# bharatlytics/faceRecognition_InfrenceEngine

Measured on AMD Instinct MI355X. Metric: faces/sec end-to-end @1080p, higher is better.
Workload: dtype f16

## Files before the change

### facerecognition_infrenceengine_amd/csrc/conv_walk64.hip

```cpp
#include "common.h"
#include <type_traits>

namespace {

constexpr int K64_RW = 28, K64_RH = 14, K64_C = 64;
constexpr int K64_PX = K64_RW * K64_RH;
constexpr int K64_HALO = 512 * 128;
constexpr int K64_SLOT = 64 * 128;
constexpr int K64_RING = 2 * K64_HALO, K64_PRMO = K64_RING + 3 * K64_SLOT;
constexpr int K64_PRM = 10 * 64 * 4;
constexpr int K64_LDS = K64_PRMO + K64_PRM;

struct Walk64P {
    const half_t* x; const half_t* w; half_t* y;
    const float* bias; const float* slope; const half_t* res;
    int B, HW, Cout, bias_mode;
    int nsplit;
    unsigned xbytes, ybytes, wbytes;
};

}

__global__ __launch_bounds__(512, 2) void conv_walk64_kernel(Walk64P p) {
#if defined(__HIP_DEVICE_COMPILE__)
    extern __shared__ __attribute__((aligned(16))) char lds[];
    char* ring = lds + K64_RING;
    float* lprm = reinterpret_cast<float*>(lds + K64_PRMO);
    const int tid = threadIdx.x;
    const int wave = __builtin_amdgcn_readfirstlane(tid >> 6);
    const int ncg = p.Cout >> 6;
    const int cg = blockIdx.x % ncg, part = (blockIdx.x / ncg) % p.nsplit, n = blockIdx.x / (ncg * p.nsplit);
    const int HW = p.HW, nbx = HW / K64_RW;
    const int reg0 = part * (nbx * (HW / K64_RH) / p.nsplit), nreg = reg0 + nbx * (HW / K64_RH) / p.nsplit;

    __amdgpu_buffer_rsrc_t wrs = buffer_rsrc(p.w, p.wbytes);
    __amdgpu_buffer_rsrc_t xrs = buffer_rsrc(p.x, p.xbytes);

    const unsigned wbase = (unsigned)cg * (9 * K64_SLOT);
    unsigned wq = 0;
    auto issue_w = [&](int slot, int ln) {
        __builtin_amdgcn_raw_ptr_buffer_load_lds(wrs, (lds_ptr_t)(ring + slot * K64_SLOT + wave * 1024), 16,
                                                 (unsigned)(wave * 1024 + ln * 16), wbase + wq * K64_SLOT, 0, 0);
        wq = wq == 8 ? 0 : wq + 1;
    };
    auto halo_lane = [&](int ln, bool left_edge, bool right_edge) -> unsigned {
        const int lrow = ln >> 3, ch = ln & 7, q = wave & 3;
        const unsigned out = (unsigned)((q == 0) & (lrow == 0) & left_edge) | (unsigned)((q == 3) & (lrow == 5) & right_edge) |
                             (unsigned)((q == 3) & (lrow >= 6));
        return ((unsigned)((lrow - 1) * 128 + ((ch ^ ((lrow + 4 * ((wave >> 2) & 1)) & 7)) << 4)) & (out - 1u)) | (out << 31);
    };
    auto issue_halo = [&](int buf, int i, int reg, int ln) {
        int n_ = n;
        asm volatile("" : "+s"(n_));
        const int by = reg / nbx, bx_ = reg - by * nbx;
        const int y0 = by * K64_RH, x0 = bx_ * K64_RW;
        const unsigned lt = halo_lane(ln, x0 == 0, x0 + K64_RW == HW);
        const int hy = 2 * i + (wave >> 2), iy = y0 - 1 + hy;
        const bool ok = reg < nreg && (unsigned)iy < (unsigned)HW;
        const unsigned so = (unsigned)(((n_ * HW + iy) * HW + x0 + (wave & 3) * 8) * 128);
        __builtin_amdgcn_raw_ptr_buffer_load_lds(xrs, (lds_ptr_t)(lds + buf * K64_HALO + (hy * 4 + (wave & 3)) * 1024), 16,
                                                 ok ? lt + so : 0x80000000u, 0, 0, 0);
    };

    {
        const int ln = tid & 63;
        issue_w(0, ln);
        issue_w(1, ln);
        issue_w(2, ln);
        for (int i = 0; i < 8; ++i) issue_halo(reg0 & 1, i, reg0, ln);
        for (int e = tid; e < 640; e += 512) {
            const int r = e >> 6, c = e & 63;
            float v;
            if (r < 9) v = p.bias ? p.bias[(p.bias_mode == 1 ? r * p.Cout : 0) + cg * 64 + c] : 0.f;
            else v = p.slope ? p.slope[cg * 64 + c] : 1.f;
            lprm[e] = v;
        }
    }

    float4v acc[3][4], accx;
    int4v a0[2][4], a1[2][4], b[3][2], bx[2];
    int boff[4];

    auto run = [&](auto role_tag) {
    constexpr int ROLE = decltype(role_tag)::value;
#pragma unroll 1
    for (int reg = reg0; reg < nreg; ++reg) {
        const int cur = reg & 1;
        int lane = tid & 63;
        asm volatile("" : "+v"(lane));
        const int fr = lane & 15, fq = lane >> 4;
        const int by = reg / nbx, bx_ = reg - by * nbx;
        const int y0 = by * K64_RH, x0 = bx_ * K64_RW;
        auto gpix = [&](int px) {
            const int oy = px / K64_RW, ox = px - oy * K64_RW;
            return (unsigned)((n * HW + y0 + oy) * HW + x0 + ox);
        };
        auto cls_off = [&](int px) {
            const int oy = px / K64_RW, ox = px - oy * K64_RW, ho = y0 + oy, wo = x0 + ox;
            return ((ho == 0 ? 0 : (ho == HW - 1 ? 2 : 1)) * 3 + (wo == 0 ? 0 : (wo == HW - 1 ? 2 : 1))) * 64;
        };
        auto ct = [&](int f) { return (f + wave) & 3; };
        auto co8 = [&](int ip) { return ct(2 * ip + (fq & 1)) * 16 + (fq >> 1) * 8; };
        int a_own = fr * 128 + ((fq ^ (fr & 7)) << 4);
        asm volatile("" : "+v"(a_own));
        int hb[3];
#pragma unroll
        for (int t = 0; t < 3; ++t) {
            const int px = (wave * 3 + t) * 16 + fr;
            const int oy = px / K64_RW, ox = px - oy * K64_RW;
            hb[t] = (oy + 1) * 32 + ox + 1;
            asm volatile("" : "+v"(hb[t]));
        }
        auto set_tap_one = [&](int t, int dy, int dx) {
            int l_ = lane;
            asm volatile("" : "+v"(l_));
            const int h = (t < 3 ? hb[t < 3 ? t : 0] : ((l_ & 15) < 8 ? 14 * 32 + 21 + (l_ & 15) : 33)) + dy * 32 + dx;
            boff[t] = cur * K64_HALO + h * 128 + (((l_ >> 4) ^ ((((h >> 3) & 4) + h) & 7)) << 4);
        };
        auto rd_a = [&](int slot, int kh, int i) { return *reinterpret_cast<const int4v*>(ring + slot * K64_SLOT + ct(i) * 2048 + (kh ? (a_own ^ 64) : a_own)); };
        auto rd_b = [&](int kh, int t) { return *reinterpret_cast<const int4v*>(lds + (kh ? (boff[t] ^ 64) : boff[t])); };

        asm volatile("s_waitcnt lgkmcnt(0)" ::: "memory");
        if (reg == reg0) __builtin_amdgcn_s_barrier();
#pragma unroll
        for (int t = 0; t < 3; ++t) {
            const int cj = cls_off((wave * 3 + t) * 16 + fr);
#pragma unroll
            for (int i = 0; i < 4; ++i) acc[t][i] = *reinterpret_cast<const float4v*>(lprm + cj + ct(i) * 16 + fq * 4);
        }
        accx = *reinterpret_cast<const float4v*>(lprm + cls_off(fr < 8 ? 384 + fr : 0) + (wave & 3) * 16 + fq * 4);
        if (p.res) {
            __amdgpu_buffer_rsrc_t rrs = buffer_rsrc(p.res, p.ybytes);
            int4v r[3][2];
#pragma unroll
            for (int t = 0; t < 3; ++t)
#pragma unroll
                for (int ip = 0; ip < 2; ++ip)
                    r[t][ip] = __builtin_bit_cast(int4v, __builtin_amdgcn_raw_buffer_load_b128(
                        rrs, (gpix((wave * 3 + t) * 16 + fr) * (unsigned)p.Cout + (unsigned)(cg * 64 + co8(ip))) * 2u, 0, 16));
            const int2v rx = __builtin_bit_cast(int2v, __builtin_amdgcn_raw_buffer_load_b64(
                rrs, fr < 8 ? (gpix(384 + fr) * (unsigned)p.Cout + (unsigned)(cg * 64 + (wave & 3) * 16 + fq * 4)) * 2u : 0x80000000u, 0, 16));
#pragma unroll
            for (int t = 0; t < 3; ++t)
#pragma unroll
                for (int ip = 0; ip < 2; ++ip) {
                    const auto s0 = __builtin_amdgcn_permlane16_swap((unsigned)r[t][ip][0], (unsigned)r[t][ip][2], false, false);
                    const auto s1 = __builtin_amdgcn_permlane16_swap((unsigned)r[t][ip][1], (unsigned)r[t][ip][3], false, false);
                    const half4 ha = __builtin_bit_cast(half4, int2v{(int)s0[0], (int)s1[0]});
                    const half4 hb_ = __builtin_bit_cast(half4, int2v{(int)s0[1], (int)s1[1]});
#pragma unroll
                    for (int e = 0; e < 4; ++e) { acc[t][2 * ip][e] += (float)ha[e]; acc[t][2 * ip + 1][e] += (float)hb_[e]; }
                }
            const half4 hx = __builtin_bit_cast(half4, rx);
#pragma unroll
            for (int e = 0; e < 4; ++e) accx[e] += (float)hx[e];
        }
        asm volatile("s_waitcnt vmcnt(0)" ::: "memory");
        __builtin_amdgcn_s_barrier();

#pragma unroll
        for (int t = 0; t < 4; ++t) set_tap_one(t, -1, -1);
#pragma unroll
        for (int kh = 0; kh < 2; ++kh) {
#pragma unroll
            for (int i = 0; i < 4; ++i) a0[kh][i] = rd_a(0, kh, i);
#pragma unroll
            for (int t = 0; t < 3; ++t) b[t][kh] = rd_b(kh, t);
            bx[kh] = rd_b(kh, 3);
        }

        auto step = [&](int4v (&ac)[2][4], int4v (&an)[2][4], int s) {
            const int nslot = (s + 1) % 3;
            const int tn = s + 1 < 9 ? s + 1 : 0;
            const int dyn = tn / 3 - 1, dxn = tn % 3 - 1;
            auto dma = [&]() {
                if (s < 8) issue_halo(cur ^ 1, s, reg + 1, lane);
                issue_w(s % 3, lane);
            };
            if constexpr (ROLE == 0) { dma(); FR_PIN(); }
#pragma unroll
            for (int kh = 0; kh < 2; ++kh) {
                accx = mfma16(ac[kh][0], bx[kh], accx);
                FR_PIN();
#pragma unroll
                for (int t = 0; t < 3; ++t) {
#pragma unroll
                    for (int i = 0; i < 4; ++i) acc[t][i] = mfma16(ac[kh][i], b[t][kh], acc[t][i]);
                    if (kh == 0) { an[0][t] = rd_a(nslot, 0, t); if (t == 2) an[0][3] = rd_a(nslot, 0, 3); }
                    else { an[1][t] = rd_a(nslot, 1, t); if (t == 2) an[1][3] = rd_a(nslot, 1, 3); }
                    if (kh == 0) set_tap_one(t, dyn, dxn);
                    b[t][kh] = rd_b(kh, t);
                    if (t == 2) {
                        if (kh == 0) set_tap_one(3, dyn, dxn);
                        bx[kh] = rd_b(kh, 3);
                    }
                    FR_PIN();
                }
                if constexpr (ROLE == 1) { if (kh == 0) { dma(); FR_PIN(); } }
            }
        };
#pragma unroll
        for (int s = 0; s < 9; ++s) {
            asm volatile("s_waitcnt vmcnt(2) lgkmcnt(1)" ::: "memory");
            __builtin_amdgcn_s_barrier();
            FR_PIN();
            if ((s & 1) == 0) step(a0, a1, s); else step(a1, a0, s);
        }

        asm volatile("s_waitcnt lgkmcnt(0)" ::: "memory");
        int le = lane;
        asm volatile("" : "+v"(le));
        const int fre = le & 15, fqe = le >> 4;
        float4v sv[4];
#pragma unroll
        for (int i = 0; i < 4; ++i) sv[i] = *reinterpret_cast<const float4v*>(lprm + 9 * 64 + ct(i) * 16 + fqe * 4);
        auto act = [&](float4v v, const float4v& s_) {
#pragma unroll
            for (int e = 0; e < 4; ++e) v[e] = v[e] > 0.f ? v[e] : v[e] * s_[e];
            return __builtin_bit_cast(int2v, half4{(half_t)v[0], (half_t)v[1], (half_t)v[2], (half_t)v[3]});
        };
        half_t* yo = p.y + cg * 64;
#pragma unroll
        for (int t = 0; t < 3; ++t) {
            const size_t gp = (size_t)gpix((wave * 3 + t) * 16 + fre) * p.Cout;
#pragma unroll
            for (int ip = 0; ip < 2; ++ip) {
                const int2v pa = act(acc[t][2 * ip], sv[2 * ip]), pb = act(acc[t][2 * ip + 1], sv[2 * ip + 1]);
                const auto s0 = __builtin_amdgcn_permlane16_swap((unsigned)pa[0], (unsigned)pb[0], false, false);
                const auto s1 = __builtin_amdgcn_permlane16_swap((unsigned)pa[1], (unsigned)pb[1], false, false);
                *reinterpret_cast<int4v*>(yo + gp + ct(2 * ip + (fqe & 1)) * 16 + (fqe >> 1) * 8) = int4v{(int)s0[0], (int)s1[0], (int)s0[1], (int)s1[1]};
            }
        }
        if (wave < 4 && fre < 8)
            *reinterpret_cast<int2v*>(yo + (size_t)gpix(384 + fre) * p.Cout + wave * 16 + fqe * 4) = act(accx, sv[0]);
    }
    };
    if ((wave >> 2) == 0) run(std::integral_constant<int, 0>{}); else run(std::integral_constant<int, 1>{});
    asm volatile("s_waitcnt vmcnt(0) lgkmcnt(0)" ::: "memory");
#endif
}

extern "C" size_t fr_conv_walk64_weight_bytes(int Cout) { return Cout > 0 ? (size_t)(Cout / 64) * 9 * K64_SLOT : 0; }

__global__ void walk64_pack_weights(const half_t* __restrict__ w, half_t* __restrict__ out, int ncg) {
    const int e = blockIdx.x * blockDim.x + threadIdx.x;
    if (e >= ncg * 9 * 512) return;
    const int q_ = e / 512, r = e - q_ * 512, row = r >> 3, cp = r & 7;
    const int cgi = q_ / 9, tap = q_ - cgi * 9;
    const int chunk = cp ^ (row & 7);
    const int4v v = *reinterpret_cast<const int4v*>(w + (size_t)(cgi * 64 + row) * 576 + tap * 64 + chunk * 8);
    *reinterpret_cast<int4v*>(out + (size_t)q_ * 4096 + row * 64 + cp * 8) = v;
}

extern "C" int fr_conv_walk64_pack(const void* w, void* out, int Cout, fr_stream_t stream) {
    FR_REQUIRE(w && out && Cout > 0 && Cout % 64 == 0, "fr_conv_walk64_pack: bad argument (Cout %d)", Cout);
    const int ncg = Cout / 64;
    walk64_pack_weights<<<fr_cdiv((int64_t)ncg * 9 * 512, 256), 256, 0, fr_stream(stream)>>>((const half_t*)w, (half_t*)out, ncg);
    FR_CHECK_LAUNCH("walk64_pack_weights");
    return FR_OK;
}

extern "C" int fr_conv_walk64_f16(const void* x, const void* wstream, void* y, const float* bias, int bias_mode, const float* slope,
                                  const void* residual, int B, int HW, int Cout, fr_stream_t stream) {
    FR_REQUIRE(x && wstream && y && B > 0, "fr_conv_walk64_f16: bad argument");
    FR_REQUIRE(x != y, "fr_conv_walk64_f16: y must not alias x");
    FR_REQUIRE(HW > 0 && HW % 28 == 0 && Cout > 0 && Cout % 64 == 0, "fr_conv_walk64_f16: image side %d must be a multiple of 28, Cout %d of 64", HW, Cout);
    FR_REQUIRE(bias_mode == 0 || bias_mode == 1, "fr_conv_walk64_f16: bad bias_mode");
    FR_REQUIRE((int64_t)B * HW * HW * 64 * 2 < (1ll << 31) && (int64_t)B * HW * HW * Cout * 2 < (1ll << 32),
               "fr_conv_walk64_f16: tensor too large for 32-bit buffer offsets (split the batch)");
    Walk64P p;
    p.x = (const half_t*)x; p.w = (const half_t*)wstream; p.y = (half_t*)y;
    p.bias = bias; p.slope = slope; p.res = (const half_t*)residual;
    p.B = B; p.HW = HW; p.Cout = Cout; p.bias_mode = bias_mode;
    const int nregs = (HW / 28) * (HW / 14);
    p.nsplit = 1;
    while (p.nsplit < 8 && (int64_t)B * (Cout / 64) * p.nsplit * 2 <= 256 && nregs % (p.nsplit * 2) == 0 && nregs / (p.nsplit * 2) >= 2) p.nsplit *= 2;
    p.xbytes = (unsigned)((int64_t)B * HW * HW * 64 * 2);
    p.ybytes = (unsigned)((int64_t)B * HW * HW * Cout * 2);
    p.wbytes = (unsigned)((int64_t)(Cout / 64) * 9 * K64_SLOT);
    static FrDevLatch latch;
    if (!fr_raise_lds(reinterpret_cast<const void*>(conv_walk64_kernel), K64_LDS, latch)) {
        fr_set_error("fr_conv_walk64_f16: cannot raise dynamic LDS to %d bytes", K64_LDS);
        return FR_E_LAUNCH;
    }
    conv_walk64_kernel<<<B * (Cout / 64) * p.nsplit, 512, K64_LDS, fr_stream(stream)>>>(p);
    FR_CHECK_LAUNCH("conv_walk64_kernel");
    return FR_OK;
}
```

Measured before the change: 26950.

## Keep conv weights resident in registers instead of streaming through LDS ring

Each wave now loads its half of the output-channel weight fragments for all 9 taps into VGPRs once at kernel start, removing the per-tap LDS weight ring, its DMA issues and the per-step barriers. Work is re-split so waves partition pixels by group (6 tiles each) and channels by half, with the extra 8 pixels handled by two pixel groups, and the weight pack layout changes to per-lane MFMA fragments. This trades a large register footprint (36 int4 per lane) for fewer LDS reads and synchronisation, which may hurt occupancy at two blocks per CU.

Result: no change. 26870 (-0.3%).

```diff
diff --git a/facerecognition_infrenceengine_amd/csrc/conv_walk64.hip b/facerecognition_infrenceengine_amd/csrc/conv_walk64.hip
--- a/facerecognition_infrenceengine_amd/csrc/conv_walk64.hip
+++ b/facerecognition_infrenceengine_amd/csrc/conv_walk64.hip
@@ -6,10 +6,11 @@
 constexpr int K64_RW = 28, K64_RH = 14, K64_C = 64;
 constexpr int K64_PX = K64_RW * K64_RH;
 constexpr int K64_HALO = 512 * 128;
-constexpr int K64_SLOT = 64 * 128;
-constexpr int K64_RING = 2 * K64_HALO, K64_PRMO = K64_RING + 3 * K64_SLOT;
+constexpr int K64_PRMO = 2 * K64_HALO;
 constexpr int K64_PRM = 10 * 64 * 4;
 constexpr int K64_LDS = K64_PRMO + K64_PRM;
+constexpr int K64_FRAG = 64 * 16;
+constexpr int K64_WCG = 4 * 9 * 2 * K64_FRAG;
 
 struct Walk64P {
     const half_t* x; const half_t* w; half_t* y;
@@ -24,25 +25,17 @@
 __global__ __launch_bounds__(512, 2) void conv_walk64_kernel(Walk64P p) {
 #if defined(__HIP_DEVICE_COMPILE__)
     extern __shared__ __attribute__((aligned(16))) char lds[];
-    char* ring = lds + K64_RING;
     float* lprm = reinterpret_cast<float*>(lds + K64_PRMO);
     const int tid = threadIdx.x;
     const int wave = __builtin_amdgcn_readfirstlane(tid >> 6);
+    const int pg = wave & 3, hf = wave >> 2;
     const int ncg = p.Cout >> 6;
     const int cg = blockIdx.x % ncg, part = (blockIdx.x / ncg) % p.nsplit, n = blockIdx.x / (ncg * p.nsplit);
     const int HW = p.HW, nbx = HW / K64_RW;
     const int reg0 = part * (nbx * (HW / K64_RH) / p.nsplit), nreg = reg0 + nbx * (HW / K64_RH) / p.nsplit;
 
-    __amdgpu_buffer_rsrc_t wrs = buffer_rsrc(p.w, p.wbytes);
     __amdgpu_buffer_rsrc_t xrs = buffer_rsrc(p.x, p.xbytes);
 
-    const unsigned wbase = (unsigned)cg * (9 * K64_SLOT);
-    unsigned wq = 0;
-    auto issue_w = [&](int slot, int ln) {
-        __builtin_amdgcn_raw_ptr_buffer_load_lds(wrs, (lds_ptr_t)(ring + slot * K64_SLOT + wave * 1024), 16,
-                                                 (unsigned)(wave * 1024 + ln * 16), wbase + wq * K64_SLOT, 0, 0);
-        wq = wq == 8 ? 0 : wq + 1;
-    };
     auto halo_lane = [&](int ln, bool left_edge, bool right_edge) -> unsigned {
         const int lrow = ln >> 3, ch = ln & 7, q = wave & 3;
         const unsigned out = (unsigned)((q == 0) & (lrow == 0) & left_edge) | (unsigned)((q == 3) & (lrow == 5) & right_edge) |
@@ -62,12 +55,20 @@
                                                  ok ? lt + so : 0x80000000u, 0, 0, 0);
     };
 
+    int4v wf[2][9][2];
     {
         const int ln = tid & 63;
-        issue_w(0, ln);
-        issue_w(1, ln);
-        issue_w(2, ln);
         for (int i = 0; i < 8; ++i) issue_halo(reg0 & 1, i, reg0, ln);
+        __amdgpu_buffer_rsrc_t wrs = buffer_rsrc(p.w, p.wbytes);
+        const unsigned wbase = (unsigned)cg * K64_WCG + (unsigned)hf * (K64_WCG / 2);
+#pragma unroll
+        for (int c = 0; c < 2; ++c)
+#pragma unroll
+            for (int tap = 0; tap < 9; ++tap)
+#pragma unroll
+                for (int kh = 0; kh < 2; ++kh)
+                    wf[c][tap][kh] = __builtin_bit_cast(int4v, __builtin_amdgcn_raw_buffer_load_b128(
+                        wrs, (unsigned)(ln * 16), wbase + (unsigned)(((c * 9 + tap) * 2 + kh) * K64_FRAG), 0));
         for (int e = tid; e < 640; e += 512) {
             const int r = e >> 6, c = e & 63;
             float v;
@@ -77,16 +78,17 @@
         }
     }
 
-    float4v acc[3][4], accx;
-    int4v a0[2][4], a1[2][4], b[3][2], bx[2];
-    int boff[4];
+    float4v acc[6][2], accx;
+    int4v b[7];
+    int boff[7];
 
     auto run = [&](auto role_tag) {
-    constexpr int ROLE = decltype(role_tag)::value;
+    constexpr int XF = decltype(role_tag)::value;
+    constexpr int NT = XF < 2 ? 7 : 6;
 #pragma unroll 1
     for (int reg = reg0; reg < nreg; ++reg) {
         const int cur = reg & 1;
-        int lane = tid & 63;
+        int lane = (int)__builtin_amdgcn_mbcnt_hi(~0u, __builtin_amdgcn_mbcnt_lo(~0u, 0u));
         asm volatile("" : "+v"(lane));
         const int fr = lane & 15, fq = lane >> 4;
         const int by = reg / nbx, bx_ = reg - by * nbx;
@@ -99,121 +101,102 @@
             const int oy = px / K64_RW, ox = px - oy * K64_RW, ho = y0 + oy, wo = x0 + ox;
             return ((ho == 0 ? 0 : (ho == HW - 1 ? 2 : 1)) * 3 + (wo == 0 ? 0 : (wo == HW - 1 ? 2 : 1))) * 64;
         };
-        auto ct = [&](int f) { return (f + wave) & 3; };
-        auto co8 = [&](int ip) { return ct(2 * ip + (fq & 1)) * 16 + (fq >> 1) * 8; };
-        int a_own = fr * 128 + ((fq ^ (fr & 7)) << 4);
-        asm volatile("" : "+v"(a_own));
-        int hb[3];
-#pragma unroll
-        for (int t = 0; t < 3; ++t) {
-            const int px = (wave * 3 + t) * 16 + fr;
+        auto co8 = [&]() { return (2 * hf + (fq & 1)) * 16 + (fq >> 1) * 8; };
+        auto tile_px = [&](int t) { return (pg * 6 + t) * 16 + fr; };
+        auto haddr = [&](int h) { return cur * K64_HALO + h * 128 + ((((h >> 3) & 4) + h) & 7) * 16; };
+        auto rd_b = [&](int t, int fx) { return *reinterpret_cast<const int4v*>(lds + (boff[t] ^ fx)); };
+
+        auto init_acc = [&](auto res_tag) {
+            constexpr bool RES = decltype(res_tag)::value;
+            int4v r[6];
+            int2v rx = {0, 0};
+            if constexpr (RES) {
+                __amdgpu_buffer_rsrc_t rrs = buffer_rsrc(p.res, p.ybytes);
+#pragma unroll
+                for (int t = 0; t < 6; ++t)
+                    r[t] = __builtin_bit_cast(int4v, __builtin_amdgcn_raw_buffer_load_b128(
+                        rrs, (gpix(tile_px(t)) * (unsigned)p.Cout + (unsigned)(cg * 64 + co8())) * 2u, 0, 16));
+                if constexpr (XF < 2)
+                    rx = __builtin_bit_cast(int2v, __builtin_amdgcn_raw_buffer_load_b64(
+                        rrs, fr < 8 ? (gpix(384 + fr) * (unsigned)p.Cout + (unsigned)(cg * 64 + (2 * hf + XF) * 16 + fq * 4)) * 2u : 0x80000000u, 0, 16));
+                FR_PIN();
+            }
+            asm volatile("s_waitcnt lgkmcnt(0)" ::: "memory");
+            if (reg == reg0) __builtin_amdgcn_s_barrier();
+            auto rd_bias = [&](int t, int c) { return *reinterpret_cast<const float4v*>(lprm + cls_off(tile_px(t)) + (2 * hf + c) * 16 + fq * 4); };
+            float4v n0 = rd_bias(0, 0), n1 = rd_bias(0, 1);
+            if constexpr (XF < 2) accx = *reinterpret_cast<const float4v*>(lprm + cls_off(fr < 8 ? 384 + fr : 0) + (2 * hf + XF) * 16 + fq * 4);
+            FR_PIN();
+#pragma unroll
+            for (int t = 0; t < 6; ++t) {
+                float4v c0 = n0, c1 = n1;
+                if (t < 5) { n0 = rd_bias(t + 1, 0); n1 = rd_bias(t + 1, 1); }
+                if constexpr (RES) {
+                    const auto s0 = __builtin_amdgcn_permlane16_swap((unsigned)r[t][0], (unsigned)r[t][2], false, false);
+                    const auto s1 = __builtin_amdgcn_permlane16_swap((unsigned)r[t][1], (unsigned)r[t][3], false, false);
+                    const half4 ha = __builtin_bit_cast(half4, int2v{(int)s0[0], (int)s1[0]});
+                    const half4 hb_ = __builtin_bit_cast(half4, int2v{(int)s0[1], (int)s1[1]});
+#pragma unroll
+                    for (int e = 0; e < 4; ++e) { c0[e] += (float)ha[e]; c1[e] += (float)hb_[e]; }
+                }
+                acc[t][0] = c0;
+                acc[t][1] = c1;
+                FR_PIN();
+            }
+            if constexpr (RES && XF < 2) {
+                const half4 hx = __builtin_bit_cast(half4, rx);
+#pragma unroll
+                for (int e = 0; e < 4; ++e) accx[e] += (float)hx[e];
+            }
+        };
+        if (p.res) init_acc(std::true_type{}); else init_acc(std::false_type{});
+#pragma unroll
+        for (int t = 0; t < NT; ++t) {
+            const int px = t < 6 ? tile_px(t) : (fr < 8 ? 384 + fr : 0);
             const int oy = px / K64_RW, ox = px - oy * K64_RW;
-            hb[t] = (oy + 1) * 32 + ox + 1;
-            asm volatile("" : "+v"(hb[t]));
-        }
-        auto set_tap_one = [&](int t, int dy, int dx) {
+            boff[t] = haddr(oy * 32 + ox);
+            asm volatile("" : "+v"(boff[t]));
+        }
+        asm volatile("s_waitcnt vmcnt(0) lgkmcnt(0)" ::: "memory");
+        __builtin_amdgcn_s_barrier();
+#pragma unroll
+        for (int t = 0; t < NT; ++t) b[t] = rd_b(t, fq << 4);
+
+        static_for<18>([&](auto ph_) {
+            constexpr int ph = decltype(ph_)::value, tap = ph >> 1, kh = ph & 1;
+            if constexpr (kh == 0 && tap < 8) { issue_halo(cur ^ 1, tap, reg + 1, lane); FR_PIN(); }
             int l_ = lane;
             asm volatile("" : "+v"(l_));
-            const int h = (t < 3 ? hb[t < 3 ? t : 0] : ((l_ & 15) < 8 ? 14 * 32 + 21 + (l_ & 15) : 33)) + dy * 32 + dx;
-            boff[t] = cur * K64_HALO + h * 128 + (((l_ >> 4) ^ ((((h >> 3) & 4) + h) & 7)) << 4);
-        };
-        auto rd_a = [&](int slot, int kh, int i) { return *reinterpret_cast<const int4v*>(ring + slot * K64_SLOT + ct(i) * 2048 + (kh ? (a_own ^ 64) : a_own)); };
-        auto rd_b = [&](int kh, int t) { return *reinterpret_cast<const int4v*>(lds + (kh ? (boff[t] ^ 64) : boff[t])); };
-
-        asm volatile("s_waitcnt lgkmcnt(0)" ::: "memory");
-        if (reg == reg0) __builtin_amdgcn_s_barrier();
-#pragma unroll
-        for (int t = 0; t < 3; ++t) {
-            const int cj = cls_off((wave * 3 + t) * 16 + fr);
-#pragma unroll
-            for (int i = 0; i < 4; ++i) acc[t][i] = *reinterpret_cast<const float4v*>(lprm + cj + ct(i) * 16 + fq * 4);
-        }
-        accx = *reinterpret_cast<const float4v*>(lprm + cls_off(fr < 8 ? 384 + fr : 0) + (wave & 3) * 16 + fq * 4);
-        if (p.res) {
-            __amdgpu_buffer_rsrc_t rrs = buffer_rsrc(p.res, p.ybytes);
-            int4v r[3][2];
-#pragma unroll
-            for (int t = 0; t < 3; ++t)
-#pragma unroll
-                for (int ip = 0; ip < 2; ++ip)
-                    r[t][ip] = __builtin_bit_cast(int4v, __builtin_amdgcn_raw_buffer_load_b128(
-                        rrs, (gpix((wave * 3 + t) * 16 + fr) * (unsigned)p.Cout + (unsigned)(cg * 64 + co8(ip))) * 2u, 0, 16));
-            const int2v rx = __builtin_bit_cast(int2v, __builtin_amdgcn_raw_buffer_load_b64(
-                rrs, fr < 8 ? (gpix(384 + fr) * (unsigned)p.Cout + (unsigned)(cg * 64 + (wave & 3) * 16 + fq * 4)) * 2u : 0x80000000u, 0, 16));
-#pragma unroll
-            for (int t = 0; t < 3; ++t)
-#pragma unroll
-                for (int ip = 0; ip < 2; ++ip) {
-                    const auto s0 = __builtin_amdgcn_permlane16_swap((unsigned)r[t][ip][0], (unsigned)r[t][ip][2], false, false);
-                    const auto s1 = __builtin_amdgcn_permlane16_swap((unsigned)r[t][ip][1], (unsigned)r[t][ip][3], false, false);
-                    const half4 ha = __builtin_bit_cast(half4, int2v{(int)s0[0], (int)s1[0]});
-                    const half4 hb_ = __builtin_bit_cast(half4, int2v{(int)s0[1], (int)s1[1]});
-#pragma unroll
-                    for (int e = 0; e < 4; ++e) { acc[t][2 * ip][e] += (float)ha[e]; acc[t][2 * ip + 1][e] += (float)hb_[e]; }
+            const int fx = (l_ & 0x30) | (kh == 0 ? 64 : 0);
+            auto next = [&](int t) {
+                if constexpr (ph < 17) {
+                    if constexpr (kh == 1) {
+                        boff[t] = ((boff[t] + (tap % 3 == 2 ? 30 * 128 : 128)) & ~0x70) | ((boff[t] + (tap % 3 == 2 ? 32 : 16)) & 0x70);
+                        asm volatile("" : "+v"(boff[t]));
+                    }
+                    b[t] = rd_b(t, fx);
                 }
-            const half4 hx = __builtin_bit_cast(half4, rx);
-#pragma unroll
-            for (int e = 0; e < 4; ++e) accx[e] += (float)hx[e];
-        }
-        asm volatile("s_waitcnt vmcnt(0)" ::: "memory");
-        __builtin_amdgcn_s_barrier();
-
-#pragma unroll
-        for (int t = 0; t < 4; ++t) set_tap_one(t, -1, -1);
-#pragma unroll
-        for (int kh = 0; kh < 2; ++kh) {
-#pragma unroll
-            for (int i = 0; i < 4; ++i) a0[kh][i] = rd_a(0, kh, i);
-#pragma unroll
-            for (int t = 0; t < 3; ++t) b[t][kh] = rd_b(kh, t);
-            bx[kh] = rd_b(kh, 3);
-        }
-
-        auto step = [&](int4v (&ac)[2][4], int4v (&an)[2][4], int s) {
-            const int nslot = (s + 1) % 3;
-            const int tn = s + 1 < 9 ? s + 1 : 0;
-            const int dyn = tn / 3 - 1, dxn = tn % 3 - 1;
-            auto dma = [&]() {
-                if (s < 8) issue_halo(cur ^ 1, s, reg + 1, lane);
-                issue_w(s % 3, lane);
             };
-            if constexpr (ROLE == 0) { dma(); FR_PIN(); }
-#pragma unroll
-            for (int kh = 0; kh < 2; ++kh) {
-                accx = mfma16(ac[kh][0], bx[kh], accx);
-                FR_PIN();
-#pragma unroll
-                for (int t = 0; t < 3; ++t) {
-#pragma unroll
-                    for (int i = 0; i < 4; ++i) acc[t][i] = mfma16(ac[kh][i], b[t][kh], acc[t][i]);
-                    if (kh == 0) { an[0][t] = rd_a(nslot, 0, t); if (t == 2) an[0][3] = rd_a(nslot, 0, 3); }
-                    else { an[1][t] = rd_a(nslot, 1, t); if (t == 2) an[1][3] = rd_a(nslot, 1, 3); }
-                    if (kh == 0) set_tap_one(t, dyn, dxn);
-                    b[t][kh] = rd_b(kh, t);
-                    if (t == 2) {
-                        if (kh == 0) set_tap_one(3, dyn, dxn);
-                        bx[kh] = rd_b(kh, 3);
-                    }
-                    FR_PIN();
-                }
-                if constexpr (ROLE == 1) { if (kh == 0) { dma(); FR_PIN(); } }
-            }
-        };
-#pragma unroll
-        for (int s = 0; s < 9; ++s) {
-            asm volatile("s_waitcnt vmcnt(2) lgkmcnt(1)" ::: "memory");
-            __builtin_amdgcn_s_barrier();
-            FR_PIN();
-            if ((s & 1) == 0) step(a0, a1, s); else step(a1, a0, s);
-        }
-
-        asm volatile("s_waitcnt lgkmcnt(0)" ::: "memory");
+            if constexpr (XF < 2) {
+                accx = mfma16(wf[XF][tap][kh], b[6], accx);
+                next(6);
+                FR_PIN();
+            }
+#pragma unroll
+            for (int t = 0; t < 6; ++t) {
+                acc[t][0] = mfma16(wf[0][tap][kh], b[t], acc[t][0]);
+                acc[t][1] = mfma16(wf[1][tap][kh], b[t], acc[t][1]);
+                next(t);
+                FR_PIN();
+            }
+        });
+
         int le = lane;
         asm volatile("" : "+v"(le));
         const int fre = le & 15, fqe = le >> 4;
-        float4v sv[4];
-#pragma unroll
-        for (int i = 0; i < 4; ++i) sv[i] = *reinterpret_cast<const float4v*>(lprm + 9 * 64 + ct(i) * 16 + fqe * 4);
+        float4v sv[2];
+#pragma unroll
+        for (int c = 0; c < 2; ++c) sv[c] = *reinterpret_cast<const float4v*>(lprm + 9 * 64 + (2 * hf + c) * 16 + fqe * 4);
         auto act = [&](float4v v, const float4v& s_) {
 #pragma unroll
             for (int e = 0; e < 4; ++e) v[e] = v[e] > 0.f ? v[e] : v[e] * s_[e];
@@ -221,41 +204,42 @@
         };
         half_t* yo = p.y + cg * 64;
 #pragma unroll
-        for (int t = 0; t < 3; ++t) {
-            const size_t gp = (size_t)gpix((wave * 3 + t) * 16 + fre) * p.Cout;
-#pragma unroll
-            for (int ip = 0; ip < 2; ++ip) {
-                const int2v pa = act(acc[t][2 * ip], sv[2 * ip]), pb = act(acc[t][2 * ip + 1], sv[2 * ip + 1]);
-                const auto s0 = __builtin_amdgcn_permlane16_swap((unsigned)pa[0], (unsigned)pb[0], false, false);
-                const auto s1 = __builtin_amdgcn_permlane16_swap((unsigned)pa[1], (unsigned)pb[1], false, false);
-                *reinterpret_cast<int4v*>(yo + gp + ct(2 * ip + (fqe & 1)) * 16 + (fqe >> 1) * 8) = int4v{(int)s0[0], (int)s1[0], (int)s0[1], (int)s1[1]};
-            }
-        }
-        if (wave < 4 && fre < 8)
-            *reinterpret_cast<int2v*>(yo + (size_t)gpix(384 + fre) * p.Cout + wave * 16 + fqe * 4) = act(accx, sv[0]);
+        for (int t = 0; t < 6; ++t) {
+            const size_t gp = (size_t)gpix((pg * 6 + t) * 16 + fre) * p.Cout;
+            const int2v pa = act(acc[t][0], sv[0]), pb = act(acc[t][1], sv[1]);
+            const auto s0 = __builtin_amdgcn_permlane16_swap((unsigned)pa[0], (unsigned)pb[0], false, false);
+            const auto s1 = __builtin_amdgcn_permlane16_swap((unsigned)pa[1], (unsigned)pb[1], false, false);
+            *reinterpret_cast<int4v*>(yo + gp + (2 * hf + (fqe & 1)) * 16 + (fqe >> 1) * 8) = int4v{(int)s0[0], (int)s1[0], (int)s0[1], (int)s1[1]};
+            FR_PIN();
+        }
+        if constexpr (XF < 2) {
+            if (fre < 8)
+                *reinterpret_cast<int2v*>(yo + (size_t)gpix(384 + fre) * p.Cout + (2 * hf + XF) * 16 + fqe * 4) = act(accx, sv[XF]);
+        }
     }
     };
-    if ((wave >> 2) == 0) run(std::integral_constant<int, 0>{}); else run(std::integral_constant<int, 1>{});
+    if (pg == 0) run(std::integral_constant<int, 0>{});
+    else if (pg == 1) run(std::integral_constant<int, 1>{});
+    else run(std::integral_constant<int, 2>{});
     asm volatile("s_waitcnt vmcnt(0) lgkmcnt(0)" ::: "memory");
 #endif
 }
 
-extern "C" size_t fr_conv_walk64_weight_bytes(int Cout) { return Cout > 0 ? (size_t)(Cout / 64) * 9 * K64_SLOT : 0; }
+extern "C" size_t fr_conv_walk64_weight_bytes(int Cout) { return Cout > 0 ? (size_t)(Cout / 64) * K64_WCG : 0; }
 
 __global__ void walk64_pack_weights(const half_t* __restrict__ w, half_t* __restrict__ out, int ncg) {
     const int e = blockIdx.x * blockDim.x + threadIdx.x;
-    if (e >= ncg * 9 * 512) return;
-    const int q_ = e / 512, r = e - q_ * 512, row = r >> 3, cp = r & 7;
-    const int cgi = q_ / 9, tap = q_ - cgi * 9;
-    const int chunk = cp ^ (row & 7);
-    const int4v v = *reinterpret_cast<const int4v*>(w + (size_t)(cgi * 64 + row) * 576 + tap * 64 + chunk * 8);
-    *reinterpret_cast<int4v*>(out + (size_t)q_ * 4096 + row * 64 + cp * 8) = v;
+    if (e >= ncg * 72 * 64) return;
+    const int f = e >> 6, ln = e & 63, fr = ln & 15, fq = ln >> 4;
+    const int cgi = f / 72, fi = f - cgi * 72, ct = fi / 18, tap = (fi - ct * 18) >> 1, kh = fi & 1;
+    const int4v v = *reinterpret_cast<const int4v*>(w + (size_t)(cgi * 64 + ct * 16 + fr) * 576 + tap * 64 + kh * 32 + fq * 8);
+    *reinterpret_cast<int4v*>(out + (size_t)e * 8) = v;
 }
 
 extern "C" int fr_conv_walk64_pack(const void* w, void* out, int Cout, fr_stream_t stream) {
     FR_REQUIRE(w && out && Cout > 0 && Cout % 64 == 0, "fr_conv_walk64_pack: bad argument (Cout %d)", Cout);
     const int ncg = Cout / 64;
-    walk64_pack_weights<<<fr_cdiv((int64_t)ncg * 9 * 512, 256), 256, 0, fr_stream(stream)>>>((const half_t*)w, (half_t*)out, ncg);
+    walk64_pack_weights<<<fr_cdiv((int64_t)ncg * 72 * 64, 256), 256, 0, fr_stream(stream)>>>((const half_t*)w, (half_t*)out, ncg);
     FR_CHECK_LAUNCH("walk64_pack_weights");
     return FR_OK;
 }
@@ -277,7 +261,7 @@
     while (p.nsplit < 8 && (int64_t)B * (Cout / 64) * p.nsplit * 2 <= 256 && nregs % (p.nsplit * 2) == 0 && nregs / (p.nsplit * 2) >= 2) p.nsplit *= 2;
     p.xbytes = (unsigned)((int64_t)B * HW * HW * 64 * 2);
     p.ybytes = (unsigned)((int64_t)B * HW * HW * Cout * 2);
-    p.wbytes = (unsigned)((int64_t)(Cout / 64) * 9 * K64_SLOT);
+    p.wbytes = (unsigned)((int64_t)(Cout / 64) * K64_WCG);
     static FrDevLatch latch;
     if (!fr_raise_lds(reinterpret_cast<const void*>(conv_walk64_kernel), K64_LDS, latch)) {
         fr_set_error("fr_conv_walk64_f16: cannot raise dynamic LDS to %d bytes", K64_LDS);
```
